# SLIDE-3D/SLIDE

Measured on AMD Instinct MI355X. Metric: latent shapes/sec (pos+feat DDPM, 1000 steps, 16 pts), higher is better.
Workload: dtype f16 (MFMA operands + activation storage; f32 accumulate, norm statistics, softmax); position DDPM: two-term f16 operand splits (fp32-grade); 1 GPU; BASELINE configs[1]+[2]: airplane position DDPM (16x3) + chair feature DDPM (16x51), batch 256 per GPU; 1 step = one reverse step of each; shape = 1000+1000 steps; batch_per_gpu=256, prec=fp16, pos_prec=split, replay=eager, pos_batch_multiple=2, pos_stream_cus=176, prime_steps=0, finite=True

## Files before the change

### include/slide_engine.h

```cpp
#ifndef SLIDE_ENGINE_H
#define SLIDE_ENGINE_H

#include <stdint.h>

#include "slide_hip.h"

#ifdef __cplusplus
extern "C" {
#endif

enum { SLIDE_EPI_RAW = 0, SLIDE_EPI_NORM = 1, SLIDE_EPI_STATS = 2 };
enum { SLIDE_F_PRE_RELU = 1, SLIDE_F_POST_RELU = 2, SLIDE_F_OUT_F32 = 4,
       SLIDE_F_RES_PAIR = 8, SLIDE_F_RES_PAIR_NBR = 16,
       SLIDE_F_OUT_FM = 32 };
enum { SLIDE_PREC_F32 = 0, SLIDE_PREC_F16 = 1, SLIDE_PREC_SPLIT = 2 };

#define SLIDE_EPI_PACKED_VECS ((uintptr_t)1)
typedef struct SlideEpi {
  int32_t mode, flags, gs, n_norm;
  float inv_count, stats_scale;
  int32_t out_ld, res_ld;
  int32_t addvec_bs, stats_bs, pre_add_ld, pre_add_shift;
  int32_t addvec_idx_stride, pad0;
  const float *bias;
// ... 52 lines not shown
};

typedef struct SlideGnFin {
  const float *sum, *sq;
  const int *gid, *gstart, *gend;
  const float *gamma, *beta;
  float *scale, *shift;
  float inv_count;
  int C, bs, G;
} SlideGnFin;

typedef struct SlidePrepCopy {
  void *dst;
  int32_t ld, kind, n, pad;
} SlidePrepCopy;

typedef struct SlideChainLayer {
  const void *X, *W, *epi;
  int32_t x_ld, k_pad, n_cob, pad;
} SlideChainLayer;

typedef struct SlideHeadArgs {
  const void *X, *W0, *W1;
  const float *v0, *b1;
  float *eps_out;
  int32_t rows, x_ld, k0, n1c, eps_ld;
  int32_t kind, C, kdim, ldf, half_out, n_copies;
  float clamp;
  uint32_t seed_lo, seed_hi;
  float *x;
  const float *noise;
  int32_t *t_dev;
  const float *keypoint, *t0, *t1, *t2, *t3, *t4, *complete_x0, *kmask;
  void *feat0;
  const struct SlidePrepCopy *copies;
} SlideHeadArgs;

typedef struct SlidePointChainArgs {
  const void *Z;
  const void *Wz;
  const void *W2;
  const void *W0, *W1;
  const float *vz;
  const float *v2;
  const float *v0, *b1;
  const float *tvec;
  const int32_t *t_idx;
  const float *cvec;
  void *X;
  float *eps;
  const void *Wz_lo, *W2_lo, *W0_lo, *W1_lo;
  int32_t rows, z_ld, kz, x_ld, k0, n1c, eps_ld, t_stride, t_bs , c_bs;
  int32_t fuse_update;
  SlideHeadArgs upd;
} SlidePointChainArgs;

typedef struct SlideOp {
  int32_t kind;
  int32_t i[11];
  float f[4];
  void *p[14];
} SlideOp;

SLIDE_API int slide_run_ops(const SlideOp *ops, int n, slide_stream_t stream);
SLIDE_API int slide_run_ops2(const SlideOp *ops, int n, slide_stream_t stream0, slide_stream_t stream1);
SLIDE_API int slide_run_chains(const SlideOp *const *ops, const int *n, const slide_stream_t *streams, int n_chains, int reps);
SLIDE_API int slide_run_chains_every(const SlideOp *const *ops, const int *n, const slide_stream_t *streams, const int *every,
                                     int n_chains, int reps);
SLIDE_API int slide_run_ops_repeat(const SlideOp *ops, int n, slide_stream_t stream0, slide_stream_t stream1, int reps);

SLIDE_API int slide_run_ops_timed(const SlideOp *ops, int n, slide_stream_t stream, float *ms_out);

SLIDE_API int slide_graph_begin(slide_stream_t stream);
SLIDE_API int slide_graph_end(slide_stream_t stream, void **graph_exec_out);
SLIDE_API int slide_graph_launch(void *graph_exec, slide_stream_t stream);
SLIDE_API int slide_graph_destroy(void *graph_exec);

SLIDE_API int slide_event_create(void **ev);
SLIDE_API int slide_event_record(void *ev, slide_stream_t stream);
SLIDE_API int slide_event_elapsed_ms(void *start, void *stop, float *ms);
SLIDE_API int slide_event_destroy(void *ev);

SLIDE_API int slide_stream_create_cu_mask(const uint32_t *mask, int n_words, slide_stream_t *stream_out);
SLIDE_API int slide_stream_destroy(slide_stream_t stream);

SLIDE_API int slide_sizeof_epi(void);
SLIDE_API int slide_sizeof_op(void);

#ifdef __cplusplus
}
#endif
#endif
```

### slide_amd/abi.py

```python
import ctypes
from ctypes import c_float, c_int32, c_uint32, c_void_p

import torch

EPI_RAW, EPI_NORM, EPI_STATS = 0, 1, 2
F_PRE_RELU, F_POST_RELU, F_OUT_F32, F_RES_PAIR, F_RES_PAIR_NBR, F_OUT_FM = 1, 2, 4, 8, 16, 32
PREC_F32, PREC_F16, PREC_SPLIT = 0, 1, 2
PREC = {"fp32": PREC_F32, "fp16": PREC_F16, "split": PREC_SPLIT}
EPI_PACKED_VECS = 1

OP_GEMM = 1
OP_PREP_POINTS = 2
OP_ASSEMBLE_SA = 3
OP_ASSEMBLE_FP = 4
OP_FINALIZE_GN = 5
OP_ATTN_COMBINE = 6
OP_COPY_COLS = 7
OP_TEMB = 8
OP_COND = 9
OP_UPDATE_POS = 10
OP_UPDATE_FEAT = 11
OP_ADVANCE_T = 12
OP_GROUPNORM_NCHW = 13
OP_SYNC = 14
# ... 13 lines not shown
OP_BLOCK_BODY = 30
OP_PAIR_FIRST = 31
OP_GEMM_CHAIN = 32
OP_HEAD_UPDATE = 33
OP_GEMM_GX_DUAL = 34
OP_SA_CHAIN_P = 35
OP_PP_STAGE = 36
OP_POINT_CHAIN = 37
OP_GEMM_ATTEND = 38
OP_ROWS_PAIR_EXPAND = 39

ST_EXPERIMENT = -20

GROUP_FP, GROUP_ABS, GROUP_CENTER, GROUP_NO_XYZ, GROUP_IDX32 = 1, 2, 4, 8, 16
GN_PRE_RELU, GN_POST_RELU, GN_STATS_ONLY, GN_APPLY_ONLY = 1, 2, 4, 8
POOL_MAX, POOL_AVG, POOL_MAX_AVG = 0, 1, 2
CHAMFER_TERM = {None: 0, "mse": 1, "cos": 2}
GEMM_LDS_DMA, GEMM_W_CM, GEMM_PAIR_RES = 1, 2, 4
TAIL_W_CM, TAIL_TWO_STAGE, TAIL_SPLIT, TAIL_FM = 1, 2, 8, 16


def _fields(ctype, names):
    return [(n, ctype) for n in names.split()]


class SlideEpi(ctypes.Structure):
    _fields_ = (_fields(c_int32, "mode flags gs n_norm") + _fields(c_float, "inv_count stats_scale")
                + _fields(c_int32, "out_ld res_ld addvec_bs stats_bs pre_add_ld pre_add_shift addvec_idx_stride pad0")
                + _fields(c_void_p, "bias gamma beta addvec addvec_idx residual pre_add out stats_sum stats_sq res_b res_vd res_vw"))


class SlideGnFin(ctypes.Structure):
    _fields_ = (_fields(c_void_p, "sum sq gid gstart gend gamma beta scale shift") + [("inv_count", c_float)]
                + _fields(c_int32, "C bs G"))


class SlidePrepCopy(ctypes.Structure):
    _fields_ = [("dst", c_void_p)] + _fields(c_int32, "ld kind n pad")


class SlideChainLayer(ctypes.Structure):
    _fields_ = _fields(c_void_p, "X W epi") + _fields(c_int32, "x_ld k_pad n_cob pad")


class SlideHeadArgs(ctypes.Structure):
    _fields_ = (_fields(c_void_p, "X W0 W1 v0 b1 eps_out")
                + _fields(c_int32, "rows x_ld k0 n1c eps_ld kind C kdim ldf half_out n_copies")
                + [("clamp", c_float), ("seed_lo", c_uint32), ("seed_hi", c_uint32)]
                + _fields(c_void_p, "x noise t_dev keypoint t0 t1 t2 t3 t4 complete_x0 kmask feat0 copies"))


class SlidePointChainArgs(ctypes.Structure):
    _fields_ = (_fields(c_void_p, "Z Wz W2 W0 W1 vz v2 v0 b1 tvec t_idx cvec X eps Wz_lo W2_lo W0_lo W1_lo")
                + _fields(c_int32, "rows z_ld kz x_ld k0 n1c eps_ld t_stride t_bs c_bs fuse_update") + [("upd", SlideHeadArgs)])


class SlideOp(ctypes.Structure):
    _fields_ = [("kind", c_int32), ("i", c_int32 * 11), ("f", c_float * 4), ("p", c_void_p * 14)]


class BodySlot(ctypes.Structure):
    _fields_ = [("src", c_void_p)] + _fields(c_int32, "chunk_stride nrows kind nvalid")


class BodyArgs(ctypes.Structure):
    _fields_ = [("slots", c_void_p), ("n_slots", c_int32),
                ("ta", c_void_p), ("tb", c_void_p),
                ("t_ld", c_int32), ("off1", c_int32), ("k1", c_int32), ("offr", c_int32), ("offk", c_int32), ("kk", c_int32),
                ("vv", c_void_p), ("vbs", c_int32), ("rv", c_void_p),
                ("nbr", c_void_p), ("d2", c_void_p), ("w", c_void_p),
                ("add0", c_void_p), ("add0_idx", c_void_p), ("add0_stride", c_int32), ("add0_bs", c_int32),
                ("sc", c_void_p), ("sh", c_void_p), ("aff_bs", c_int32),
                ("P", c_void_p), ("p_ld", c_int32),
                ("vec1", c_void_p), ("n1", c_int32), ("gs1", c_int32), ("inv1", c_float),
                ("add1", c_void_p), ("add1_bs", c_int32),
                ("vecm", c_void_p), ("n_mo", c_int32), ("gsm", c_int32), ("invm", c_float),
                ("addm", c_void_p), ("addm_bs", c_int32),
                ("vecu", c_void_p), ("n_u", c_int32), ("gsu", c_int32), ("nnu", c_int32), ("invu", c_float),
                ("vect", c_void_p), ("n_out", c_int32), ("gsv", c_int32), ("nnv", c_int32), ("invv", c_float),
                ("out", c_void_p), ("out_ld", c_int32), ("out2", c_void_p), ("out2_ld", c_int32), ("out2_n", c_int32),
                ("B", c_int32), ("dbg", c_void_p)]


UNCHECKED_STRUCTS = ("BodySlot", "BodyArgs")

_CTYPE = {"i": ctypes.c_int, "q": ctypes.c_longlong, "f": c_float, "p": c_void_p}


def _proto(args, restype=ctypes.c_int):
    return restype, tuple(_CTYPE[a] for a in args)


PROTOTYPES = {name: _proto(args) for name, args in {
    "gather_points_kernel_wrapper": "iiiipppp",
    "gather_points_grad_kernel_wrapper": "iiiipppp",
    "furthest_point_sampling_kernel_wrapper": "iiipppp",
    "query_ball_point_kernel_wrapper": "iiifippppp",
    "group_points_kernel_wrapper": "iiiiipppp",
    "group_points_grad_kernel_wrapper": "iiiiipppp",
    "three_nn_kernel_wrapper": "iiippppp",
    "three_interpolate_kernel_wrapper": "iiiippppp",
    "three_interpolate_grad_kernel_wrapper": "iiiippppp",
    "slide_knn_points": "iiiipppppp",
    "slide_knn_gather": "iiiiipppp",
    "slide_sample_farthest_points": "iiippppp",
    "slide_gather_rows": "iiiipppp",
    "slide_chamfer_nn": "iiipipippppppp",
# ... 100 lines not shown
```

### slide_amd/csrc/point_chain.hip

```cpp
#include "gemm_common.h"
#include "ddpm_update.h"
#include "launch.h"

namespace {

typedef SlidePointChainArgs ChainArgs;

template <int KZMAX, int K0MAX, bool WIDE>
__global__ __launch_bounds__(256, 1) void point_chain_kernel(ChainArgs a) {
#pragma clang fp contract(off)
  using T = _Float16;
  constexpr int LDZ = KZMAX + 8, LDH = 128 + 8, LDX = K0MAX + 8;
  __shared__ __attribute__((aligned(16))) T zs[32 * LDZ];
  __shared__ __attribute__((aligned(16))) T hs[32 * LDH];
  __shared__ __attribute__((aligned(16))) T xs[32 * LDX];
  __shared__ __attribute__((aligned(16))) T hs_lo[WIDE ? 32 * LDH : 8];
  __shared__ __attribute__((aligned(16))) T xs_lo[WIDE ? 32 * LDX : 8];
  constexpr int NVL = 512 + 256 + 384 + 256 + 384 + 64;
  __shared__ __attribute__((aligned(16))) float vl[NVL];
  float *const vz_l = vl, *const tv_l = vl + 512, *const v2_l = vl + 768, *const cv_l = vl + 1152, *const v0_l = vl + 1408,
        *const bo_l = vl + 1792;
  const int tid = threadIdx.x, lane = tid & 63, wave = tid >> 6, half = lane >> 5, col = lane & 31;
  const int row0 = blockIdx.x * 32;
  const int nkz = a.kz >> 4, nk0 = a.k0 >> 4;
  f16x8 wz[2][KZMAX / 16], w2[8], w0[K0MAX / 16], w1[8];
  f16x8 wzl[2][WIDE ? KZMAX / 16 : 1], w2l[WIDE ? 8 : 1];
  if constexpr (WIDE) {
    const GLOBAL_AS T *wp = gptr<const T>((uint64_t)a.Wz_lo) + (size_t)(wave * 32 + col) * a.kz + half * 8;
#pragma unroll
    for (int s2 = 0; s2 < KZMAX / 16; ++s2)
      if (s2 < nkz) {
        wzl[0][s2] = *(const GLOBAL_AS f16x8 *)(wp + s2 * 16);
        wzl[1][s2] = *(const GLOBAL_AS f16x8 *)(wp + (size_t)128 * a.kz + s2 * 16);
      }
    const GLOBAL_AS T *w2p = gptr<const T>((uint64_t)a.W2_lo) + (size_t)(wave * 32 + col) * 128 + half * 8;
#pragma unroll
    for (int s2 = 0; s2 < 8; ++s2) w2l[s2] = *(const GLOBAL_AS f16x8 *)(w2p + s2 * 16);
  }
  {
    const GLOBAL_AS T *wp = gptr<const T>((uint64_t)a.Wz) + (size_t)(wave * 32 + col) * a.kz + half * 8;
#pragma unroll
    for (int s2 = 0; s2 < KZMAX / 16; ++s2)
      if (s2 < nkz) {
        wz[0][s2] = *(const GLOBAL_AS f16x8 *)(wp + s2 * 16);
        wz[1][s2] = *(const GLOBAL_AS f16x8 *)(wp + (size_t)128 * a.kz + s2 * 16);
      }
    const GLOBAL_AS T *w2p = gptr<const T>((uint64_t)a.W2) + (size_t)(wave * 32 + col) * 128 + half * 8;
#pragma unroll
    for (int s2 = 0; s2 < 8; ++s2) w2[s2] = *(const GLOBAL_AS f16x8 *)(w2p + s2 * 16);
    const GLOBAL_AS T *w0p = gptr<const T>((uint64_t)a.W0) + (size_t)(wave * 32 + col) * a.k0 + half * 8;
#pragma unroll
    for (int s2 = 0; s2 < K0MAX / 16; ++s2)
      if (s2 < nk0) w0[s2] = *(const GLOBAL_AS f16x8 *)(w0p + s2 * 16);
    if (wave < a.n1c) {
      const GLOBAL_AS T *w1p = gptr<const T>((uint64_t)a.W1) + (size_t)(wave * 32 + col) * 128 + half * 8;
#pragma unroll
      for (int s2 = 0; s2 < 8; ++s2) w1[s2] = *(const GLOBAL_AS f16x8 *)(w1p + s2 * 16);
    }
  }
  {
    const int ppr = a.kz >> 3;
    for (int i = tid; i < 32 * ppr; i += 256) {
      const int r = i / ppr, pc = i - r * ppr;
      int grow = row0 + r;
      grow = grow < a.rows ? grow : a.rows - 1;
      *reinterpret_cast<u32x4 *>(zs + r * LDZ + pc * 8) = *(const GLOBAL_AS u32x4 *)(gptr<const T>((uint64_t)a.Z) + (size_t)grow * a.z_ld + pc * 8);
    }
    const int ppx = (a.k0 - 128) >> 3;
    for (int i = tid; i < 32 * ppx; i += 256) {
      const int r = i / ppx, pc = i - r * ppx;
      int grow = row0 + r;
      grow = grow < a.rows ? grow : a.rows - 1;
      *reinterpret_cast<u32x4 *>(xs + r * LDX + 128 + pc * 8) =
          *(const GLOBAL_AS u32x4 *)(gptr<const T>((uint64_t)a.X) + (size_t)grow * a.x_ld + 128 + pc * 8);
      if constexpr (WIDE) *reinterpret_cast<u32x4 *>(xs_lo + r * LDX + 128 + pc * 8) = u32x4{0, 0, 0, 0};
    }
    const int nsm = a.rows >> 4, smp0 = row0 >> 4;
    for (int i = tid; i < NVL; i += 256) {
      float v = 0.f;
      if (i < 512) v = a.vz[i];
      else if (i < 768) {
        int sm = smp0 + ((i - 512) >> 7);
        sm = sm < nsm ? sm : nsm - 1;
        if (a.tvec) v = a.tvec[(a.t_idx ? (size_t)a.t_idx[0] * a.t_stride : 0) + (size_t)sm * a.t_bs + ((i - 512) & 127)];
      } else if (i < 1152) v = a.v2[i - 768];
      else if (i < 1408) {
        int sm = smp0 + ((i - 1152) >> 7);
        sm = sm < nsm ? sm : nsm - 1;
        if (a.cvec) v = a.cvec[(size_t)sm * a.c_bs + ((i - 1152) & 127)];
      } else if (i < 1792) v = a.v0[i - 1408];
      else if (i - 1792 < a.n1c * 32) v = a.b1[i - 1792];
      vl[i] = v;
    }
  }
  __shared__ float zl[32 * 64];
  int ut = 0, ustep = 0;
  uint32_t unonce = 0, ueoff = 0;
  if (a.fuse_update) {
    const SlideHeadArgs &u = a.upd;
    ut = u.t_dev[0]; ustep = u.t_dev[1];
    unonce = (uint32_t)u.t_dev[3];
    ueoff = (uint32_t)u.t_dev[4] * (uint32_t)(16 * u.C);
    if (ut > 0)
      for (int i = tid; i < 32 * u.C; i += 256) {
        const int r = i / u.C, c = i - r * u.C, p = row0 + r;
        if (c < u.kdim || p >= a.rows) continue;
        const int e = p * u.C + c;
        zl[r * 64 + c] = u.noise ? u.noise[(size_t)ustep * a.rows * u.C + e]
                                 : philox_normal(u.seed_lo, u.seed_hi, (uint32_t)ustep, (uint32_t)e + ueoff, unonce);
      }
  }
  __syncthreads();
  auto vec16 = [&](const float *base, float (&o)[16]) __attribute__((always_inline)) {
#pragma unroll
    for (int q = 0; q < 4; ++q) {
      const float4 t4 = *reinterpret_cast<const float4 *>(base + wave * 32 + 8 * q + 4 * half);
      o[4 * q] = t4.x; o[4 * q + 1] = t4.y; o[4 * q + 2] = t4.z; o[4 * q + 3] = t4.w;
    }
  };
  auto gn_relu = [&](const f32x16 &acc, const float *vec3, float (&y)[16]) __attribute__((always_inline)) {
    float bia[16], gam[16], bet[16];
    vec16(vec3, bia); vec16(vec3 + 128, gam); vec16(vec3 + 256, bet);
#pragma unroll
    for (int q = 0; q < 4; ++q) {
      float v[4], s = 0.f, ss = 0.f;
#pragma unroll
      for (int j = 0; j < 4; ++j) {
        v[j] = acc[4 * q + j] + bia[4 * q + j];
        s += v[j];
        ss = fmaf(v[j], v[j], ss);
      }
      s = lane_group_sum<16>(s);
      ss = lane_group_sum<16>(ss);
      const float mean = s * (1.0f / 64.0f);
      const float var = fmaxf(ss * (1.0f / 64.0f) - mean * mean, 0.f);
      const float rstd = __builtin_amdgcn_rsqf(var + GN_EPS);
#pragma unroll
      for (int j = 0; j < 4; ++j) {
        const float g = gam[4 * q + j] * rstd;
        y[4 * q + j] = fmaxf(fmaf(v[j], g, bet[4 * q + j] - mean * g), 0.f);
      }
    }
  };
  auto put16 = [&](T *dst_row, const float (&y)[16]) __attribute__((always_inline)) {
#pragma unroll
    for (int q = 0; q < 4; ++q) {
      f16x4 h;
#pragma unroll
      for (int j = 0; j < 4; ++j) h[j] = (T)y[4 * q + j];
      *reinterpret_cast<f16x4 *>(dst_row + wave * 32 + 8 * q + 4 * half) = h;
    }
  };
  auto put16w = [&](T *hi_row, T *lo_row, const float (&y)[16]) __attribute__((always_inline)) {
#pragma unroll
    for (int q = 0; q < 4; ++q) {
      f16x4 h, l;
#pragma unroll
      for (int j = 0; j < 4; ++j) {
        h[j] = (T)y[4 * q + j];
        l[j] = (T)((y[4 * q + j] - (float)h[j]) * 2048.0f);
      }
      *reinterpret_cast<f16x4 *>(hi_row + wave * 32 + 8 * q + 4 * half) = h;
      *reinterpret_cast<f16x4 *>(lo_row + wave * 32 + 8 * q + 4 * half) = l;
    }
  };
  auto zero16 = [](f32x16 &v) __attribute__((always_inline)) {
#pragma unroll
    for (int r = 0; r < 16; ++r) v[r] = 0.f;
  };
  auto fold = [](f32x16 &hi, const f32x16 &lo) __attribute__((always_inline)) {
#pragma unroll
    for (int r = 0; r < 16; ++r) hi[r] = fmaf(lo[r], 1.0f / 2048.0f, hi[r]);
  };
  f32x16 ah, ar;
  zero16(ah); zero16(ar);
  {
    f32x16 al, arl;
    if constexpr (WIDE) { zero16(al); zero16(arl); }
#pragma unroll
    for (int s2 = 0; s2 < KZMAX / 16; ++s2)
      if (s2 < nkz) {
        const f16x8 xb = *reinterpret_cast<const f16x8 *>(zs + col * LDZ + s2 * 16 + half * 8);
        ah = __builtin_amdgcn_mfma_f32_32x32x16_f16(wz[0][s2], xb, ah, 0, 0, 0);
        ar = __builtin_amdgcn_mfma_f32_32x32x16_f16(wz[1][s2], xb, ar, 0, 0, 0);
        if constexpr (WIDE) {
          al = __builtin_amdgcn_mfma_f32_32x32x16_f16(wzl[0][s2], xb, al, 0, 0, 0);
          arl = __builtin_amdgcn_mfma_f32_32x32x16_f16(wzl[1][s2], xb, arl, 0, 0, 0);
        }
      }
    if constexpr (WIDE) { fold(ah, al); fold(ar, arl); }
  }
  f16x8 w0l[WIDE ? K0MAX / 16 : 1], w1l[WIDE ? 8 : 1];
  if constexpr (WIDE) {
    const GLOBAL_AS T *w0p = gptr<const T>((uint64_t)a.W0_lo) + (size_t)(wave * 32 + col) * a.k0 + half * 8;
#pragma unroll
    for (int s2 = 0; s2 < K0MAX / 16; ++s2)
      if (s2 < nk0) w0l[s2] = *(const GLOBAL_AS f16x8 *)(w0p + s2 * 16);
    if (wave < a.n1c) {
      const GLOBAL_AS T *w1p = gptr<const T>((uint64_t)a.W1_lo) + (size_t)(wave * 32 + col) * 128 + half * 8;
#pragma unroll
      for (int s2 = 0; s2 < 8; ++s2) w1l[s2] = *(const GLOBAL_AS f16x8 *)(w1p + s2 * 16);
    }
  }
  float res[16];
  {
    float y[16], tv[16], br[16];
    gn_relu(ah, vz_l, y);
    vec16(tv_l + (col >> 4) * 128, tv); vec16(vz_l + 384, br);
#pragma unroll
    for (int r = 0; r < 16; ++r) { y[r] += tv[r]; res[r] = ar[r] + br[r]; }
    if constexpr (WIDE) put16w(hs + col * LDH, hs_lo + col * LDH, y);
    else put16(hs + col * LDH, y);
  }
  __syncthreads();
  {
    f32x16 a2, a2l;
    zero16(a2);
    if constexpr (WIDE) zero16(a2l);
#pragma unroll
    for (int s2 = 0; s2 < 8; ++s2) {
      const f16x8 hb = *reinterpret_cast<const f16x8 *>(hs + col * LDH + s2 * 16 + half * 8);
      a2 = __builtin_amdgcn_mfma_f32_32x32x16_f16(w2[s2], hb, a2, 0, 0, 0);
      if constexpr (WIDE) {
        const f16x8 hl = *reinterpret_cast<const f16x8 *>(hs_lo + col * LDH + s2 * 16 + half * 8);
        a2l = __builtin_amdgcn_mfma_f32_32x32x16_f16(w2[s2], hl, a2l, 0, 0, 0);
        a2l = __builtin_amdgcn_mfma_f32_32x32x16_f16(w2l[s2], hb, a2l, 0, 0, 0);
      }
    }
    if constexpr (WIDE) fold(a2, a2l);
    float y[16], cv[16];
    gn_relu(a2, v2_l, y);
    vec16(cv_l + (col >> 4) * 128, cv);
#pragma unroll
    for (int r = 0; r < 16; ++r) y[r] = y[r] + cv[r] + res[r];
    if constexpr (WIDE) put16w(xs + col * LDX, xs_lo + col * LDX, y);
    else put16(xs + col * LDX, y);
    if (row0 + col < a.rows) put16(reinterpret_cast<T *>(a.X) + (size_t)(row0 + col) * a.x_ld, y);
  }
  __syncthreads();
  {
    f32x16 a3, a3l;
    zero16(a3);
    if constexpr (WIDE) zero16(a3l);
#pragma unroll
    for (int s2 = 0; s2 < K0MAX / 16; ++s2)
      if (s2 < nk0) {
// ... 14 lines not shown
  __syncthreads();
  if (wave < a.n1c) {
    f32x16 e2, e2l;
    zero16(e2);
    if constexpr (WIDE) zero16(e2l);
#pragma unroll
    for (int s2 = 0; s2 < 8; ++s2) {
      const f16x8 hb = *reinterpret_cast<const f16x8 *>(hs + col * LDH + s2 * 16 + half * 8);
      e2 = __builtin_amdgcn_mfma_f32_32x32x16_f16(w1[s2], hb, e2, 0, 0, 0);
      if constexpr (WIDE) {
        const f16x8 hl = *reinterpret_cast<const f16x8 *>(hs_lo + col * LDH + s2 * 16 + half * 8);
        e2l = __builtin_amdgcn_mfma_f32_32x32x16_f16(w1[s2], hl, e2l, 0, 0, 0);
        e2l = __builtin_amdgcn_mfma_f32_32x32x16_f16(w1l[s2], hb, e2l, 0, 0, 0);
      }
    }
    if constexpr (WIDE) fold(e2, e2l);
    float bo[16];
#pragma unroll
    for (int q = 0; q < 4; ++q) {
      const float4 t4 = *reinterpret_cast<const float4 *>(bo_l + wave * 32 + 8 * q + 4 * half);
      bo[4 * q] = t4.x; bo[4 * q + 1] = t4.y; bo[4 * q + 2] = t4.z; bo[4 * q + 3] = t4.w;
    }
    const int p = row0 + col;
    if (p < a.rows) {
#pragma unroll
      for (int q = 0; q < 4; ++q) {
        const int c = wave * 32 + 8 * q + 4 * half;
        if (a.eps && c + 3 < a.eps_ld)
          *reinterpret_cast<float4 *>(a.eps + (size_t)p * a.eps_ld + c) =
              make_float4(e2[4 * q] + bo[4 * q], e2[4 * q + 1] + bo[4 * q + 1], e2[4 * q + 2] + bo[4 * q + 2], e2[4 * q + 3] + bo[4 * q + 3]);
      }
      if (a.fuse_update) {
        const SlideHeadArgs &u = a.upd;
#pragma unroll
        for (int r = 0; r < 16; ++r) {
          const int c = wave * 32 + (r & 3) + 8 * (r >> 2) + 4 * half;
          if (c >= u.C) continue;
          update_feat_element(p * u.C + c, a.rows, u.C, u.kdim, 0, u.clamp, u.seed_lo, u.seed_hi, u.x, nullptr, u.noise, ut, ustep, unonce,
                              ueoff, u.complete_x0, u.kmask, u.keypoint, u.t0, u.t1, u.t2, u.t3, u.t4, u.feat0, u.ldf, u.half_out,
                              u.copies, u.n_copies, e2[r] + bo[r], zl + col * 64 + c);
        }
      }
    }
  }
  if (a.fuse_update) advance_t_last_block(a.upd.t_dev, ut, ustep);
}

}

int slide_launch_point_chain(const SlideOp &o, hipStream_t s) {
  const SlidePointChainArgs *h = (const SlidePointChainArgs *)o.p[0];
  if (!h || h->rows <= 0 || h->rows % 16 || h->kz % 32 || h->kz <= 0 || h->kz > 192 || h->z_ld < h->kz || h->z_ld % 8 || h->k0 % 32 ||
      h->k0 <= 128 || h->k0 > 160 || h->x_ld < h->k0 || h->x_ld % 8 || (h->n1c != 1 && h->n1c != 2) || h->eps_ld % 4 ||
      h->eps_ld > 32 * h->n1c || h->t_bs < 0 || !h->Z || !h->Wz || !h->W2 || !h->W0 || !h->W1 || !h->vz || !h->v2 || !h->v0 || !h->b1 || !h->X || (!h->eps && !h->fuse_update))
    return -3;
  if (h->fuse_update && (h->upd.kind != 1 || h->upd.C > 32 * h->n1c || h->upd.C > 64 || !h->upd.x || !h->upd.t_dev || !h->upd.t0 || !h->upd.t1 ||
                         !h->upd.t2 || !h->upd.t3 || !h->upd.t4 || (h->upd.kdim > 0 && !h->upd.keypoint)))
    return -3;
  const bool wide = h->Wz_lo || h->W2_lo || h->W0_lo || h->W1_lo;
  if (wide && !(h->Wz_lo && h->W2_lo && h->W0_lo && h->W1_lo)) return -3;
  if (wide) hipLaunchKernelGGL((point_chain_kernel<192, 160, true>), dim3((h->rows + 31) / 32), dim3(256), 0, s, *h);
  else hipLaunchKernelGGL((point_chain_kernel<192, 160, false>), dim3((h->rows + 31) / 32), dim3(256), 0, s, *h);
  return (int)hipGetLastError();
}
```

### slide_amd/engine.py

```python
import ctypes
from typing import NamedTuple

import numpy as np
import torch

from . import knobs
from ._lib import SlideHipError, check, lib
from .abi import *


class GnLayout(NamedTuple):
    index: np.ndarray
    width: int
    n_norm: int
    gs: int
    gs_logical: int

    @classmethod
    def plain(cls, C):
        return cls(np.arange(C), C, 0, 1, 1)

    @property
    def unpermuted(self):
        return np.array_equal(self.index, np.arange(len(self.index)))

    @property
    def identity(self):
        return self.unpermuted and self.width == len(self.index) and self.n_norm == len(self.index)

    def raw(self):
        return GnLayout(self.index, self.width, 0, 1, 1)


def gn_layout(C):
    G = min(32, C)
    n_norm = C - C % G
    gs = n_norm // G
    gs_p = 1
    while gs_p < gs:
        gs_p *= 2
    assert gs_p <= 32, "GroupNorm group size > 32 not supported by the epilogue"
    idx = np.empty(C, np.int64)
    for c in range(C):
        idx[c] = (c // gs) * gs_p + c % gs if c < n_norm else G * gs_p + (c - n_norm)
    return GnLayout(idx, int(G * gs_p + (C - n_norm)), int(G * gs_p), int(gs_p), int(gs))


class AddVec(NamedTuple):
    vec: torch.Tensor
    off: int
    bs: int
    idx: torch.Tensor = None
    idx_stride: int = 0


class PreAdd(NamedTuple):
    table: torch.Tensor
    shift: int
    coff: int = 0
# ... 1116 lines not shown
        hz, rz = self._buf(B * 16, n1), self._buf(B * 16, n2)
        f2, r2 = self._mlp_segments(m2, self.tvec, hz, rz)
        i0 = len(self.plan)
        self._gemm(Z, 4, [f2, r2])
        out = out_buf if out_buf is not None else self._buf(B * 16, n2)
        self._mlp_tail(m2, 4, hz, self.cvec, rz, out)
        if out_buf is not None:
            self._chain_front = ChainFront(self.plan[i0:], Z, zin, m2, n1, n2)
        return out, n2

    def _head_arrays(self, k0):
        sd, w0, w1 = self.sd, self._w("fc_lyaer.0.weight"), self._w("fc_lyaer.3.weight")
        lay0, n1c = gn_layout(w0.shape[0]), ru(self.out_dim) // 32
        if not (self.prec == 1 and w0.shape[0] == 128 and lay0.identity and lay0.gs == 4 and k0 <= 160 and w1.shape[1] == 128
                and self.out_dim <= 64 and sd["fc_lyaer.1.weight"].shape[0] == 128):
            return None
        W0 = np.zeros((128, k0), np.float32); W0[:, :w0.shape[1]] = w0
        W1 = np.zeros((n1c * 32, 128), np.float32); W1[:w1.shape[0]] = w1
        b1 = np.zeros(n1c * 32, np.float32); b1[:w1.shape[0]] = sd["fc_lyaer.3.bias"]
        return W0, W1, b1, epi_vectors(lay0, 128, sd["fc_lyaer.0.bias"], (sd["fc_lyaer.1.weight"], sd["fc_lyaer.1.bias"])), n1c

    def _point_chain(self, dec0, head):
        sd, fr = self.sd, getattr(self, "_chain_front", None)
        hd = self._head_arrays(dec0.shape[1])
        if fr is None or hd is None or not self.knobs.SLIDE_POINT_CHAIN:
            return None
        m2, lay = fr.m2, gn_layout(128)
        c2 = sd[m2 + ".second_mlp.0.weight"].shape[0]
        has_t, has_c = (m2 + ".fc.weight") in sd, (m2 + ".fc_condition.weight") in sd
        if not (fr.n1 == 128 and fr.n2 == 128 and c2 == 128 and (m2 + ".rest_mlp.0.weight") not in sd and lay.identity and lay.gs == 4
                and len(fr.launches) == 2 and self.plan[-4:] == fr.launches + head and fr.Z.shape[1] <= 192 and 128 < dec0.shape[1]):
            return None
        A, kz, zin = self.A, fr.Z.shape[1], fr.zin
        Wz = np.zeros((256, kz), np.float32)
        Wz[:128, :zin] = self._w(m2 + ".first_mlp.0.weight")
        Wz[128:, :zin] = self._w(m2 + ".res_connect.weight")
        vz = np.stack([sd[m2 + ".first_mlp.0.bias"], sd[m2 + ".first_mlp.1.group_norm.weight"], sd[m2 + ".first_mlp.1.group_norm.bias"],
                       sd[m2 + ".res_connect.bias"]]).astype(np.float32)
        v2 = epi_vectors(lay, 128, sd[m2 + ".second_mlp.0.bias"], (sd[m2 + ".second_mlp.1.group_norm.weight"],
                                                                   sd[m2 + ".second_mlp.1.group_norm.bias"]))
        (W0, W1, b1, v0, n1c), W2 = hd, self._w(m2 + ".second_mlp.0.weight")
        off = lambda lst, pfx: sum(w for _, w in lst[:[p_ for p_, _ in lst].index(pfx)])
        for role, e in zip(("pc0", "pc1", "pc2", "pc3"), self.plan[-4:]):
            e.roles.add(role)
        d = dict(Z=fr.Z, kz=kz, X=dec0, k0=dec0.shape[1], n1c=n1c,
                 Wz=A.put(Wz, torch.float16), W2=A.put(W2, torch.float16),
                 W0=A.put(W0, torch.float16), W1=A.put(W1, torch.float16), vz=A.put(vz), v2=A.put(v2), v0=A.put(v0), b1=A.put(b1),
                 t_off=off(self._tvec, m2 + ".fc") if has_t else None,
                 c_off=off(self._cvec, m2 + ".fc_condition") if has_c else None)
        if self.knobs.SLIDE_POINT_CHAIN_WIDE:
            def lo(w):
                w = np.asarray(w, np.float32)
                return ((w - w.astype(np.float16).astype(np.float32)) * np.float32(2048.0)).astype(np.float32)
            d.update(Wz_lo=A.put(lo(Wz), torch.float16), W2_lo=A.put(lo(W2), torch.float16), W0_lo=A.put(lo(W0), torch.float16),
                     W1_lo=A.put(lo(W1), torch.float16))
        return d

    def point_chain_args(self, eps_out=None):
        pch = getattr(self, "point_chain", None)
        if pch is None:
            return None
        c = SlidePointChainArgs()
        for k_ in ("Z", "Wz", "W2", "W0", "W1", "vz", "v2", "v0", "b1", "X", "Wz_lo", "W2_lo", "W0_lo", "W1_lo"):
            if k_ in pch:
                setattr(c, k_, pch[k_].data_ptr())
        c.eps = (eps_out if eps_out is not None else self.eps_pad).data_ptr()
        c.rows, c.z_ld, c.kz, c.x_ld, c.k0, c.n1c = self.B * 16, pch["Z"].shape[1], pch["kz"], pch["X"].shape[1], pch["k0"], pch["n1c"]
        c.eps_ld = self.eps_pad.shape[1]
        if pch["t_off"] is not None:
            c.tvec = self.tvec.data_ptr() + 4 * pch["t_off"]
            if self.per_sample_t:
                c.t_idx, c.t_stride, c.t_bs = None, 0, self._t_bs
            else:
                c.t_idx, c.t_stride, c.t_bs = self.t_dev.data_ptr(), self._n_fc, 0
        if pch["c_off"] is not None:
            c.cvec, c.c_bs = self.cvec.data_ptr() + 4 * pch["c_off"], self._c_bs
        return c

    def _build(self):
        hp, sd, B, A = self.hp, self.sd, self.B, self.A
        arch = hp["architecture"]
        self.persistent = self.knobs.SLIDE_PERSISTENT
        self.x = A.zeros(B, 16, self.cx)
        self.ts = A.zeros(B)
        self.label = A.zeros(B, dtype=torch.int64)
        self.t_dev = A.zeros(8, dtype=torch.int32)
        self.xyz = A.zeros(B * 16, 3)
        C0 = self.cx
        self.feat0 = self._buf(B * 16, C0)
        self.kidx = A.zeros(B * 16, 16, dtype=torch.int32)
        self.kd2 = A.zeros(B * 16, 16)
        self.kw = A.zeros(B * 16, 16)
        n_fc = sum(v.shape[0] for k, v in sd.items() if k.endswith(".fc.weight"))
        n_fcc = sum(v.shape[0] for k, v in sd.items() if k.endswith(".fc_condition.weight"))
        self._n_fc = n_fc
        self._t_bs = n_fc if self.per_sample_t else 0
        self._c_bs = n_fcc
        self.tvec = A.zeros(B if self.per_sample_t else self.t_table, n_fc)
        self.cvec = A.zeros(B, n_fcc)
        temb_slot = None
        if self.per_sample_t:
            temb_slot = Launch(None)
            self.plan.append(temb_slot)
        feat0_cm = None
        if self.use_cm and self.knobs.SLIDE_CM_TABLES:
            feat0_cm = self._cm_copy[self.feat0.data_ptr()] = self._buf(B * 16, C0)
        self.fold_copies = self.knobs.SLIDE_FOLD_COPIES
        self._prep_copies, self._tail_of = [], {}
        prep = self._emit(make_op(OP_PREP_POINTS, i=(B, self.cx, self.feat0.shape[1], self.prec),
                                  p=(self.x.data_ptr(), self.xyz.data_ptr(), self.feat0.data_ptr(), self.kidx.data_ptr(),
                                     self.kd2.data_ptr(), _dp(feat0_cm), None, self.kw.data_ptr())), role="prep").op
        feats, chans = [self.feat0], [C0]
        nsa, nfp = len(arch["npoint"]), len(arch["decoder_feature_dim"]) - 1
        fp_q = {}
        for i in range(nsa):
            j = i + nfp - nsa
            extra = ()
            if 0 <= j < nfp and self.knobs.SLIDE_MERGE_Q:
# ... 217 lines not shown
```

### slide_amd/knobs.py

```python
import os
from typing import NamedTuple, Optional


class Knob(NamedTuple):
    name: str
    kind: str
    default: Optional[str]
    scope: str
    doc: str


_PARSE = {"flag": lambda s: s != "0", "int": int, "float": float, "text": lambda s: s, "opt": lambda s: s}


def _table(scope, rows):
    return [Knob(n, k, d, scope, doc) for n, k, d, doc in rows]


TABLE = _table("plan", [
    ("SLIDE_GLDS", "flag", "1", "fp16 plans use the LDS-DMA ring kernels (0: the register-staged kernel for every GEMM)"),
    ("SLIDE_GLDS_WIDE", "int", "0", "1: 64-deep K chunks (row-major operands), 2: eight-wave 256x256 tiles, 3: no split-K small-launch "
                                    "kernel, 4: eight-wave narrow tiles"),
    ("SLIDE_CM", "flag", "1", "chunk-major activations and weights for the 128- / 256-row ring kernels (0: row-major everywhere)"),
    ("SLIDE_CM_TABLES", "flag", "0", "chunk-major second copies of the gathered per-point tables as well"),
    ("SLIDE_GX", "flag", "1", "pair decomposition of the blocks' first layers + generated-X GEMMs (0: first layers over gathered inputs)"),
    ("SLIDE_GXS", "flag", "1", "split plans: the pair decomposition in the split arithmetic (0: the fp32-structured plan)"),
    ("SLIDE_XS", "text", "", "X-stationary GEMM kernel: \"\" off, \"auto\", or the row-tile log2 sizes \"7,8\"; any value turns "
                             "chunk-major storage off"),
    ("SLIDE_XS_CBW", "text", "2", "X-stationary kernel: \"4\" = four-block column tiles"),
    ("SLIDE_XS_OCC", "opt", None, "X-stationary kernel: cap on its workgroups per CU (empty: no cap)"),
    ("SLIDE_TWO_LANES", "flag", "0", "score / value branches of an attention block on two streams"),
    ("SLIDE_FM", "flag", "1", "u / mo of the register-X attention tails stored fragment-major (0: chunk-major)"),
    ("SLIDE_ATTN_TAIL", "flag", "1", "scores + values + soft-max + sum in the fused attention tail (0: two GEMMs + combine launch)"),
    ("SLIDE_TAIL_SPLIT", "flag", "1", "split plans: the same tail in the split arithmetic (0: two GEMMs + combine launch)"),
    ("SLIDE_TAIL_OCC3", "flag", "0", "attention tail: two-stage ring at three workgroups per CU"),
    ("SLIDE_TAIL_WIDE", "opt", None, "attention tail: four-wave 256x128 form for layers of at least this many channel blocks; set at "
                                     "all, it turns fragment-major storage off"),
    ("SLIDE_BODY", "text", "0", "\"0\": three launches per block; otherwise the one-launch block body for FP0-sized blocks, \"2\": "
                                "for SA0 too"),
    ("SLIDE_PACKED_VECS", "flag", "1", "descriptor buffers carry [bias | gamma | beta] behind the descriptors, pointer bit 0 says so "
                                       "(0: plain pointer); the module path reads it too, per call"),
    ("SLIDE_CBW4_TILES", "int", "1000", "minimum tile count for 128-channel tiles"),
    ("SLIDE_CBW1_TILES", "int", "0", "maximum tile count for 32-channel tiles"),
    ("SLIDE_STAGGER_US", "float", "0", "start stagger of the odd wave slot; A/B switches ride on the same field"),
    ("SLIDE_PERSISTENT", "int", "0", "1: tile counter per XCD, 2: static tile lists"),
    ("SLIDE_GX_N64", "text", "1", "generated-X GEMMs on 64-channel tiles (\"0\": 128-channel tiles)"),
    ("SLIDE_GX_N64W", "flag", "1", "64-channel tiles at two workgroups per CU where the 128-channel grid would leave CUs empty"),
    ("SLIDE_GX_DUAL", "flag", "1", "the mode-1 and mode-0 generated-X GEMMs of an FP block in one launch (0: two launches)"),
    ("SLIDE_GXS_CHAIN", "flag", "1", "split plans: second_mlp -> rest_mlp of an SA block in one launch"),
    ("SLIDE_SA_CHAIN", "flag", "1", "SA second_mlp -> rest_mlp in one launch with h2 in registers"),
    ("SLIDE_CHAIN_P", "flag", "1", "SA blocks: query GEMM + Mlp chain in one launch (0: apart)"),
    ("SLIDE_PAIR_FUSED", "flag", "1", "per-point GEMM + pair-table pass in one launch (0: GEMM -> fp32 y -> pair-norm launch)"),
    ("SLIDE_PAIR_NORM_V2", "flag", "0", "one 1024-thread workgroup per sample finalises the joint GroupNorm too"),
    ("SLIDE_SPLIT_FIRST", "int", "1000000", "minimum feature width for evaluating a block's first layer per point"),
    ("SLIDE_FUSE_FIN", "flag", "1", "GroupNorm finalisation of the score branch folded into the per-point query GEMM"),
    ("SLIDE_GATHER", "flag", "1", "first GEMM of an SA / FP block DMA-gathers the neighbour rows (0: grouped input assembled in memory)"),
    ("SLIDE_MERGE_Q", "flag", "1", "attention queries ride on a shared per-point GEMM (0: one query GEMM per attention block)"),
    ("SLIDE_FOLD_COPIES", "flag", "1", "COPY launches folded into the producers of their sources (0: separate launches)"),
    ("SLIDE_GEMM_CHAIN", "int", "0", "largest chain (KB of weights) of consecutive per-point GEMMs merged into one launch"),
    ("SLIDE_PP", "flag", "0", "split plans: runs of 16-row launches as one per-point stage launch"),
    ("SLIDE_POINT_CHAIN", "flag", "1", "FP0's second Mlp + the output head offered to the samplers as one launch (0: four launches)"),
    ("SLIDE_POINT_CHAIN_WIDE", "flag", "1", "the point chain in the split arithmetic (0: fp16 operands)"),
    ("SLIDE_FUSE_PREP", "flag", "1", "feature sampler: point preparation once per chain (0: one launch per step)"),
    ("SLIDE_HEAD_UPDATE", "flag", "0", "output head + DDPM update in one launch"),
    ("SLIDE_POINT_CHAIN_UPDATE", "flag", "0", "the feature DDPM's update rides on the point-chain launch too"),
    ("SLIDE_ABL_DROP", "opt", None, "TIMING ablation: launches whose kernel name contains one of these substrings are left out"),
    ("SLIDE_STREAM_PRIO", "opt", None, "\"<position>,<feature>\" HIP stream priorities of the chains (-1 high)"),
    ("SLIDE_POS_CUS", "opt", None, "compute units the position chains' streams may use (0 = all)"),
    ("SLIDE_FEAT_CUS", "opt", None, "compute units the feature chains' streams may use (0 = all)"),
    ("SLIDE_CU_MASK_FROM", "int", "0", "first compute unit of those masks"),
]) + _table("live", [
    ("SLIDE_MODULE_PREC", "text", "fp32", "module path: \"fp16\" = fp16 MFMA operands, fp32 accumulate"),
    ("SLIDE_MODULE_STATS", "flag", "1", "module path: GroupNorm statistics from the producing GEMM's epilogue"),
    ("SLIDE_MODULE_DEFER", "flag", "1", "module path: deferred normalisation (fp16 operands only)"),
    ("SLIDE_MODULE_PAIR", "flag", "1", "fp16 module path: convolutions over grouped inputs by the pair decomposition"),
    ("SLIDE_MODULE_FUSE_ATTEND", "flag", "1", "fp16 module path: score GEMM + soft-max + weighted sum in one launch"),
    ("SLIDE_MODULE_SPLIT_QK", "flag", "1", "fp16 module path: AttentionModule without the [q | k] concatenation"),
    ("SLIDE_MODULE_CBW4", "flag", "0", "module path: 128-channel tiles"),
    ("SLIDE_PINNED_TABLES", "flag", "1", "module path: descriptor tables through pinned slots + asynchronous copies"),
    ("SLIDE_POS_MULT", "int", "2", "generation: the position chain runs over this multiple of the batch"),
    ("SLIDE_SHARE_GPU", "flag", "0", "generation CLIs: all ranks on device 0 over gloo"),
    ("SLIDE_HIP_LIB", "opt", None, "path of an alternative libslide_hip.so (read by _lib.py at import)"),
    ("SLIDE_EXPERIMENTS", "text", "0", "anything but \"\" and \"0\": load the experiments library (read by _lib.py at import)"),
    ("SLIDE_ALLOW_SPILLS", "flag", "0", "a spilling kernel in the product build is a warning, not an error (read by build.py)"),
]) + _table("library", [
    ("SLIDE_TAIL_RX", "flag", "1", "fp16 attention tails load their X fragments straight into registers (0: the LDS-ring form)"),
    ("SLIDE_TAIL8", "flag", "0", "eight-wave 256x128 attention tail"),
    ("SLIDE_TAIL_ABL", "opt", None, "attention tail timing ablations (tools only)"),
    ("SLIDE_SA_SPLIT", "opt", None, "0: the SA chain never runs on two workgroups per sample"),
    ("SLIDE_SA_SPLIT_MAX", "opt", None, "launches of at most this many samples run the SA chain on two workgroups per sample"),
    ("SLIDE_XS_NSPLIT", "opt", None, "X-stationary kernel: cap on its column split"),
])
KNOBS = {k.name: k for k in TABLE}
assert len(KNOBS) == len(TABLE)


def read(name):
    k = KNOBS[name]
    return _PARSE[k.kind](os.environ.get(name, k.default))


Snapshot = NamedTuple("Snapshot", [(k.name, object) for k in TABLE if k.scope != "live"])


def snapshot():
    return Snapshot(*map(read, Snapshot._fields))


if __name__ == "__main__":
    for k in TABLE:
        print("%-26s %-8s default %-9s now %-9r %s" % (k.name, k.scope, k.default, read(k.name), k.doc))
```

Measured before the change: 436.2 shapes/s.

## Pack point-chain weights into contiguous per-wave MFMA fragment buffer

Adds a host-side packer that reorders the point chain's four weight matrices (and their low-order split halves) into one buffer of per-wave MFMA fragments, so each lane loads a contiguous 16-byte piece per fragment. A packed variant of the kernel loads weights with fully coalesced loads and interleaves the Z/X/vector prologue loads with the weight loads using scheduling barriers. It is meant to cut the strided row-major weight fetch cost and hide prologue latency in a launch that runs every step. It adds a new ABI field, a default-on knob, and a fixed k0=160 requirement for the packed path.

After: 442.9 shapes/s (median of 6 runs). +1.5%, better.

```diff
diff --git a/include/slide_engine.h b/include/slide_engine.h
--- a/include/slide_engine.h
+++ b/include/slide_engine.h
@@ -128,6 +128,7 @@
   const void *Wz_lo, *W2_lo, *W0_lo, *W1_lo;
   int32_t rows, z_ld, kz, x_ld, k0, n1c, eps_ld, t_stride, t_bs , c_bs;
   int32_t fuse_update;
+  int32_t wpk_bytes;
   SlideHeadArgs upd;
 } SlidePointChainArgs;
 
diff --git a/slide_amd/abi.py b/slide_amd/abi.py
--- a/slide_amd/abi.py
+++ b/slide_amd/abi.py
@@ -89,7 +89,8 @@
 
 class SlidePointChainArgs(ctypes.Structure):
     _fields_ = (_fields(c_void_p, "Z Wz W2 W0 W1 vz v2 v0 b1 tvec t_idx cvec X eps Wz_lo W2_lo W0_lo W1_lo")
-                + _fields(c_int32, "rows z_ld kz x_ld k0 n1c eps_ld t_stride t_bs c_bs fuse_update") + [("upd", SlideHeadArgs)])
+                + _fields(c_int32, "rows z_ld kz x_ld k0 n1c eps_ld t_stride t_bs c_bs fuse_update wpk_bytes")
+                + [("upd", SlideHeadArgs)])
 
 
 class SlideOp(ctypes.Structure):
diff --git a/slide_amd/chain_pack.py b/slide_amd/chain_pack.py
--- /dev/null
+++ b/slide_amd/chain_pack.py
@@ -0,0 +1,40 @@
+import numpy as np
+
+FRAG = 512
+
+
+def fragment(W, w, s):
+    return W[32 * w:32 * w + 32, 16 * s:16 * s + 16].reshape(32, 2, 8).transpose(1, 0, 2).reshape(-1)
+
+
+def n_fragments(kz, k0, n1c, wide):
+    return (4 * (2 * (kz // 16) + 8 + k0 // 16) + 8 * n1c) * (2 if wide else 1)
+
+
+def wave_order(kz, k0, n1c, w, wide):
+    out = []
+    for s in range(kz // 16):
+        out += [("Wz", 0, s), ("Wz", 128, s)] + ([("Wz_lo", 0, s), ("Wz_lo", 128, s)] if wide else [])
+    out += [("W2", 0, s) for s in range(8)] + ([("W2_lo", 0, s) for s in range(8)] if wide else [])
+    out += [("W0", 0, s) for s in range(k0 // 16)]
+    if w < n1c:
+        out += [("W1", 0, s) for s in range(8)]
+    if wide:
+        out += [("W0_lo", 0, s) for s in range(k0 // 16)]
+        if w < n1c:
+            out += [("W1_lo", 0, s) for s in range(8)]
+    return out
+
+
+def pack(Wz, W2, W0, W1, lo=None):
+    m = dict(Wz=Wz, W2=W2, W0=W0, W1=W1)
+    if lo is not None:
+        m.update(zip(("Wz_lo", "W2_lo", "W0_lo", "W1_lo"), lo))
+    m = {k: np.ascontiguousarray(v, np.float16) for k, v in m.items()}
+    kz, k0, n1c = m["Wz"].shape[1], m["W0"].shape[1], m["W1"].shape[0] // 32
+    assert m["Wz"].shape == (256, kz) and kz % 32 == 0 and m["W2"].shape == (128, 128) and m["W0"].shape == (128, k0) and k0 % 16 == 0
+    assert m["W1"].shape == (32 * n1c, 128) and all(m[k + "_lo"].shape == m[k].shape for k in ("Wz", "W2", "W0", "W1") if lo is not None)
+    out = [fragment(m[name][r0:], w, s) for w in range(4) for name, r0, s in wave_order(kz, k0, n1c, w, lo is not None)]
+    out = np.concatenate(out)
+    assert out.size == FRAG * n_fragments(kz, k0, n1c, lo is not None)
+    return out
diff --git a/slide_amd/csrc/point_chain.hip b/slide_amd/csrc/point_chain.hip
--- a/slide_amd/csrc/point_chain.hip
+++ b/slide_amd/csrc/point_chain.hip
@@ -6,7 +6,7 @@
 
 typedef SlidePointChainArgs ChainArgs;
 
-template <int KZMAX, int K0MAX, bool WIDE>
+template <int KZMAX, int K0MAX, bool WIDE, bool PACKED>
 __global__ __launch_bounds__(256, 1) void point_chain_kernel(ChainArgs a) {
 #pragma clang fp contract(off)
   using T = _Float16;
@@ -25,6 +25,113 @@
   const int nkz = a.kz >> 4, nk0 = a.k0 >> 4;
   f16x8 wz[2][KZMAX / 16], w2[8], w0[K0MAX / 16], w1[8];
   f16x8 wzl[2][WIDE ? KZMAX / 16 : 1], w2l[WIDE ? 8 : 1];
+  const uint32_t lane16 = lane * 16;
+  const GLOBAL_AS char *wpk_head = nullptr;
+  if constexpr (PACKED) {
+    constexpr int LW = WIDE ? 4 : 2, N2 = WIDE ? 16 : 8, ZPT = KZMAX * 4 / 256;
+    static_assert((K0MAX - 128) * 4 <= 256 && ZPT * 256 == KZMAX * 4, "one piece of the head's extra columns per thread");
+    const int wave_s = __builtin_amdgcn_readfirstlane(wave);
+    const bool has1 = wave_s < a.n1c;
+    constexpr int NK0 = K0MAX / 16;
+    const int o2 = nkz * LW, o1 = o2 + N2 + NK0, oh = o1 + (has1 ? 8 : 0), per_wave = o1 + (WIDE ? NK0 : 0);
+    const GLOBAL_AS char *wb = gptr<const char>((uint64_t)a.Wz) + ((size_t)(wave_s * per_wave + (has1 ? wave_s : a.n1c) * N2) << 10);
+    wpk_head = wb + ((size_t)oh << 10);
+    auto frag = [&](int f, bool live) __attribute__((always_inline)) {
+      const GLOBAL_AS char *p = wb + (live ? (size_t)f << 10 : (size_t)0);
+      return *(const GLOBAL_AS f16x8 *)(p + (live ? lane16 : 0u));
+    };
+    const int trow = a.t_idx ? a.t_idx[0] : 0;
+    const int ppr = a.kz >> 3, ppx = (a.k0 - 128) >> 3, nsm = a.rows >> 4, smp0 = row0 >> 4;
+    u32x4 zr[ZPT], xr;
+    int zdst[ZPT];
+#pragma unroll
+    for (int j = 0; j < ZPT; ++j) {
+      const int i = tid + 256 * j;
+      const bool ok = i < 32 * ppr;
+      const int ii = ok ? i : 0, r = ii / ppr, pc = ii - r * ppr;
+      int grow = row0 + r;
+      grow = grow < a.rows ? grow : a.rows - 1;
+      zr[j] = *(const GLOBAL_AS u32x4 *)(gptr<const T>((uint64_t)a.Z) + (size_t)grow * a.z_ld + pc * 8);
+      zdst[j] = ok ? r * LDZ + pc * 8 : -1;
+    }
+    int xdst;
+    {
+      const bool ok = tid < 32 * ppx;
+      const int ii = ok ? tid : 0, r = ii / ppx, pc = ii - r * ppx;
+      int grow = row0 + r;
+      grow = grow < a.rows ? grow : a.rows - 1;
+      xr = *(const GLOBAL_AS u32x4 *)(gptr<const T>((uint64_t)a.X) + (size_t)grow * a.x_ld + 128 + pc * 8);
+      xdst = ok ? r * LDX + 128 + pc * 8 : -1;
+    }
+    float vr[8];
+    bool vok[8];
+    {
+      const uint64_t pvz = (uint64_t)a.vz, pv2 = (uint64_t)a.v2, pv0 = (uint64_t)a.v0, pb1 = (uint64_t)a.b1, pcv = (uint64_t)a.cvec;
+      const bool lo128 = tid < 128, hc = pcv != 0, hb = tid < a.n1c * 32;
+      const int s0 = smp0 < nsm ? smp0 : nsm - 1, s1 = smp0 + 1 < nsm ? smp0 + 1 : nsm - 1;
+      const uint64_t c0 = hc ? pcv + 4 * ((uint64_t)s0 * a.c_bs + (tid & 127)) : pvz;
+      const uint64_t c1 = hc ? pcv + 4 * ((uint64_t)s1 * a.c_bs + (tid & 127)) : pvz;
+      const uint64_t src[8] = {pvz + 4 * tid, pvz + 4 * (tid + 256), 0, pv2 + 4 * tid, lo128 ? pv2 + 4 * (tid + 256) : c0,
+                               lo128 ? c1 : pv0 + 4 * (tid - 128), pv0 + 4 * (tid + 128), hb ? pb1 + 4 * tid : pvz};
+      const bool okj[8] = {true, true, false, true, lo128 || hc, !lo128 || hc, true, hb};
+#pragma unroll
+      for (int j = 0; j < 8; ++j)
+        if (j != 2) {
+          vr[j] = *gptr<const float>(src[j]);
+          vok[j] = okj[j];
+        }
+    }
+    auto issue_l1 = [&](int s2) __attribute__((always_inline)) {
+      const bool live = s2 < nkz;
+      wz[0][s2] = frag(s2 * LW, live);
+      wz[1][s2] = frag(s2 * LW + 1, live);
+      if constexpr (WIDE) {
+        wzl[0][s2] = frag(s2 * LW + 2, live);
+        wzl[1][s2] = frag(s2 * LW + 3, live);
+      }
+    };
+    __builtin_amdgcn_sched_barrier(0);
+#pragma unroll
+    for (int s2 = 0; s2 < KZMAX / 32; ++s2) issue_l1(s2);
+    __builtin_amdgcn_sched_barrier(0);
+#pragma unroll
+    for (int j = 0; j < ZPT; ++j)
+      if (zdst[j] >= 0) *reinterpret_cast<u32x4 *>(zs + zdst[j]) = zr[j];
+    if (xdst >= 0) {
+      *reinterpret_cast<u32x4 *>(xs + xdst) = xr;
+      if constexpr (WIDE) *reinterpret_cast<u32x4 *>(xs_lo + xdst) = u32x4{0, 0, 0, 0};
+    }
+#pragma unroll
+    for (int j = 0; j < 8; ++j)
+      if (j != 2 && tid + 256 * j < NVL) vl[tid + 256 * j] = vok[j] ? vr[j] : 0.f;
+    __builtin_amdgcn_sched_barrier(0);
+    float tv;
+    {
+      int sm = smp0 + (tid >> 7);
+      sm = sm < nsm ? sm : nsm - 1;
+      const uint64_t pt = (uint64_t)a.tvec;
+      tv = *gptr<const float>(pt ? pt + 4 * ((a.t_idx ? (uint64_t)trow * a.t_stride : 0) + (uint64_t)sm * a.t_bs + (tid & 127)) : (uint64_t)a.vz);
+    }
+#pragma unroll
+    for (int s2 = KZMAX / 32; s2 < KZMAX / 16; ++s2) issue_l1(s2);
+    {
+      const GLOBAL_AS char *b2 = wb + ((size_t)o2 << 10);
+#pragma unroll
+      for (int s2 = 0; s2 < 8; ++s2) w2[s2] = *(const GLOBAL_AS f16x8 *)(b2 + s2 * 1024 + lane16);
+      if constexpr (WIDE) {
+#pragma unroll
+        for (int s2 = 0; s2 < 8; ++s2) w2l[s2] = *(const GLOBAL_AS f16x8 *)(b2 + (8 + s2) * 1024 + lane16);
+      }
+#pragma unroll
+      for (int s2 = 0; s2 < NK0; ++s2) w0[s2] = *(const GLOBAL_AS f16x8 *)(b2 + (N2 + s2) * 1024 + lane16);
+      const GLOBAL_AS char *b1 = wb + (has1 ? ((size_t)o1 << 10) : (size_t)0);
+      const uint32_t vo1 = has1 ? lane16 : 0u;
+#pragma unroll
+      for (int s2 = 0; s2 < 8; ++s2) w1[s2] = *(const GLOBAL_AS f16x8 *)(b1 + (has1 ? s2 * 1024 : 0) + vo1);
+    }
+    __builtin_amdgcn_sched_barrier(0);
+    vl[512 + tid] = a.tvec ? tv : 0.f;
+  } else {
   if constexpr (WIDE) {
     const GLOBAL_AS T *wp = gptr<const T>((uint64_t)a.Wz_lo) + (size_t)(wave * 32 + col) * a.kz + half * 8;
 #pragma unroll
@@ -93,6 +200,7 @@
       vl[i] = v;
     }
   }
+  }
   __shared__ float zl[32 * 64];
   int ut = 0, ustep = 0;
   uint32_t unonce = 0, ueoff = 0;
@@ -191,7 +299,15 @@
     if constexpr (WIDE) { fold(ah, al); fold(ar, arl); }
   }
   f16x8 w0l[WIDE ? K0MAX / 16 : 1], w1l[WIDE ? 8 : 1];
-  if constexpr (WIDE) {
+  if constexpr (WIDE && PACKED) {
+    __builtin_amdgcn_sched_barrier(0);
+    const bool has1 = __builtin_amdgcn_readfirstlane(wave) < a.n1c;
+    const uint32_t vo1 = has1 ? lane16 : 0u;
+#pragma unroll
+    for (int s2 = 0; s2 < K0MAX / 16; ++s2) w0l[s2] = *(const GLOBAL_AS f16x8 *)(wpk_head + s2 * 1024 + lane16);
+#pragma unroll
+    for (int s2 = 0; s2 < 8; ++s2) w1l[s2] = *(const GLOBAL_AS f16x8 *)(wpk_head + (has1 ? (K0MAX / 16 + s2) * 1024 : 0) + vo1);
+  } else if constexpr (WIDE) {
     const GLOBAL_AS T *w0p = gptr<const T>((uint64_t)a.W0_lo) + (size_t)(wave * 32 + col) * a.k0 + half * 8;
 #pragma unroll
     for (int s2 = 0; s2 < K0MAX / 16; ++s2)
@@ -312,14 +428,26 @@
   const SlidePointChainArgs *h = (const SlidePointChainArgs *)o.p[0];
   if (!h || h->rows <= 0 || h->rows % 16 || h->kz % 32 || h->kz <= 0 || h->kz > 192 || h->z_ld < h->kz || h->z_ld % 8 || h->k0 % 32 ||
       h->k0 <= 128 || h->k0 > 160 || h->x_ld < h->k0 || h->x_ld % 8 || (h->n1c != 1 && h->n1c != 2) || h->eps_ld % 4 ||
-      h->eps_ld > 32 * h->n1c || h->t_bs < 0 || !h->Z || !h->Wz || !h->W2 || !h->W0 || !h->W1 || !h->vz || !h->v2 || !h->v0 || !h->b1 || !h->X || (!h->eps && !h->fuse_update))
+      h->eps_ld > 32 * h->n1c || h->t_bs < 0 || !h->Z || !h->Wz || !h->vz || !h->v2 || !h->v0 || !h->b1 || !h->X || (!h->eps && !h->fuse_update))
     return -3;
   if (h->fuse_update && (h->upd.kind != 1 || h->upd.C > 32 * h->n1c || h->upd.C > 64 || !h->upd.x || !h->upd.t_dev || !h->upd.t0 || !h->upd.t1 ||
                          !h->upd.t2 || !h->upd.t3 || !h->upd.t4 || (h->upd.kdim > 0 && !h->upd.keypoint)))
     return -3;
+  const dim3 grid((h->rows + 31) / 32);
+  if (h->wpk_bytes) {
+    const int frags = 4 * (2 * (h->kz / 16) + 8 + h->k0 / 16) + 8 * h->n1c;
+    const bool wide = h->wpk_bytes == 2048 * frags;
+    if ((!wide && h->wpk_bytes != 1024 * frags) || h->k0 != 160 || ((uintptr_t)h->Wz & 15) || h->W2 || h->W0 || h->W1 || h->Wz_lo || h->W2_lo || h->W0_lo ||
+        h->W1_lo)
+      return -3;
+    if (wide) hipLaunchKernelGGL((point_chain_kernel<192, 160, true, true>), grid, dim3(256), 0, s, *h);
+    else hipLaunchKernelGGL((point_chain_kernel<192, 160, false, true>), grid, dim3(256), 0, s, *h);
+    return (int)hipGetLastError();
+  }
+  if (!h->W2 || !h->W0 || !h->W1) return -3;
   const bool wide = h->Wz_lo || h->W2_lo || h->W0_lo || h->W1_lo;
   if (wide && !(h->Wz_lo && h->W2_lo && h->W0_lo && h->W1_lo)) return -3;
-  if (wide) hipLaunchKernelGGL((point_chain_kernel<192, 160, true>), dim3((h->rows + 31) / 32), dim3(256), 0, s, *h);
-  else hipLaunchKernelGGL((point_chain_kernel<192, 160, false>), dim3((h->rows + 31) / 32), dim3(256), 0, s, *h);
+  if (wide) hipLaunchKernelGGL((point_chain_kernel<192, 160, true, false>), grid, dim3(256), 0, s, *h);
+  else hipLaunchKernelGGL((point_chain_kernel<192, 160, false, false>), grid, dim3(256), 0, s, *h);
   return (int)hipGetLastError();
 }
diff --git a/slide_amd/engine.py b/slide_amd/engine.py
--- a/slide_amd/engine.py
+++ b/slide_amd/engine.py
@@ -4,7 +4,7 @@
 import numpy as np
 import torch
 
-from . import knobs
+from . import chain_pack, knobs
 from ._lib import SlideHipError, check, lib
 from .abi import *
 
@@ -1227,8 +1227,13 @@
             def lo(w):
                 w = np.asarray(w, np.float32)
                 return ((w - w.astype(np.float16).astype(np.float32)) * np.float32(2048.0)).astype(np.float32)
-            d.update(Wz_lo=A.put(lo(Wz), torch.float16), W2_lo=A.put(lo(W2), torch.float16), W0_lo=A.put(lo(W0), torch.float16),
-                     W1_lo=A.put(lo(W1), torch.float16))
+            los = [lo(w) for w in (Wz, W2, W0, W1)]
+            d.update(Wz_lo=A.put(los[0], torch.float16), W2_lo=A.put(los[1], torch.float16), W0_lo=A.put(los[2], torch.float16),
+                     W1_lo=A.put(los[3], torch.float16))
+        else:
+            los = None
+        if self.knobs.SLIDE_POINT_CHAIN_PACKED:
+            d["Wpk"] = A.put(chain_pack.pack(Wz, W2, W0, W1, los))
         return d
 
     def point_chain_args(self, eps_out=None):
@@ -1236,9 +1241,12 @@
         if pch is None:
             return None
         c = SlidePointChainArgs()
-        for k_ in ("Z", "Wz", "W2", "W0", "W1", "vz", "v2", "v0", "b1", "X", "Wz_lo", "W2_lo", "W0_lo", "W1_lo"):
+        packed = "Wpk" in pch
+        for k_ in ("Z", "vz", "v2", "v0", "b1", "X") + (() if packed else ("Wz", "W2", "W0", "W1", "Wz_lo", "W2_lo", "W0_lo", "W1_lo")):
             if k_ in pch:
                 setattr(c, k_, pch[k_].data_ptr())
+        if packed:
+            c.Wz, c.wpk_bytes = pch["Wpk"].data_ptr(), pch["Wpk"].numel() * 2
         c.eps = (eps_out if eps_out is not None else self.eps_pad).data_ptr()
         c.rows, c.z_ld, c.kz, c.x_ld, c.k0, c.n1c = self.B * 16, pch["Z"].shape[1], pch["kz"], pch["X"].shape[1], pch["k0"], pch["n1c"]
         c.eps_ld = self.eps_pad.shape[1]
diff --git a/slide_amd/knobs.py b/slide_amd/knobs.py
--- a/slide_amd/knobs.py
+++ b/slide_amd/knobs.py
@@ -61,6 +61,7 @@
     ("SLIDE_PP", "flag", "0", "split plans: runs of 16-row launches as one per-point stage launch"),
     ("SLIDE_POINT_CHAIN", "flag", "1", "FP0's second Mlp + the output head offered to the samplers as one launch (0: four launches)"),
     ("SLIDE_POINT_CHAIN_WIDE", "flag", "1", "the point chain in the split arithmetic (0: fp16 operands)"),
+    ("SLIDE_POINT_CHAIN_PACKED", "flag", "1", "the point chain reads its weights as one buffer of packed MFMA fragments (0: row-major)"),
     ("SLIDE_FUSE_PREP", "flag", "1", "feature sampler: point preparation once per chain (0: one launch per step)"),
     ("SLIDE_HEAD_UPDATE", "flag", "0", "output head + DDPM update in one launch"),
     ("SLIDE_POINT_CHAIN_UPDATE", "flag", "0", "the feature DDPM's update rides on the point-chain launch too"),
```
